# moribots/plen_ml_walk

Measured on NVIDIA B200. Metric: PLEN env-steps/sec, higher is better.
Workload: dtype f32

## Files before the change

### plen_ml_walk_b200/csrc/plen_device.cuh

```cuda
#pragma once

#include <math.h>
#include <stdint.h>

#include "../../include/plen_b200.h"

#ifndef PLEN_HOST_EMU
#define PLEN_DEV __device__ __forceinline__
#define PLEN_DEV_NOINLINE __device__ __noinline__
namespace plen {
PLEN_DEV int lane_id() { return threadIdx.x & 31; }
PLEN_DEV float shfl(float v, int src) { return __shfl_sync(0xffffffffu, v, src); }
PLEN_DEV float shfl4(float v, int src) { return __shfl_sync(0xffffffffu, v, src, 4); }
PLEN_DEV float shfl_up(float v, int d) { return __shfl_up_sync(0xffffffffu, v, d); }
PLEN_DEV float shfl_down(float v, int d) { return __shfl_down_sync(0xffffffffu, v, d); }
PLEN_DEV float shfl_xor(float v, int m) { return __shfl_xor_sync(0xffffffffu, v, m); }
PLEN_DEV unsigned ballot(bool p) { return __ballot_sync(0xffffffffu, p); }
PLEN_DEV unsigned redux_max(unsigned v) { return __reduce_max_sync(0xffffffffu, v); }
PLEN_DEV unsigned redux_or(unsigned v) { return __reduce_or_sync(0xffffffffu, v); }
PLEN_DEV void warp_sync() { __syncwarp(); }
PLEN_DEV float f_as_u_max(float v) { return __uint_as_float(redux_max(__float_as_uint(v))); }
PLEN_DEV void sincos_(float x, float *s, float *c) { sincosf(x, s, c); }
#ifndef PLEN_FAST_RCP
#define PLEN_FAST_RCP 1
#endif
PLEN_DEV float rcp_(float x) {
#if PLEN_FAST_RCP
    float r;
    asm("rcp.approx.ftz.f32 %0, %1;" : "=f"(r) : "f"(x));
    return r;
#else
    return 1.0f / x;
#endif
}
PLEN_DEV unsigned f_bits(float v) { return __float_as_uint(v); }
PLEN_DEV int lowest_bit(unsigned m) { return __ffs((int)m) - 1; }
PLEN_DEV int highest_bit(unsigned m) { return 31 - __clz((int)m); }
PLEN_DEV int popc_(unsigned m) { return __popc(m); }
}
#endif

namespace plen {

enum {
    T_RPJ = 0, T_PPJ = 9, T_AXIS = 12, T_COM = 15, T_MASS = 18, T_INERTIA = 19, T_LOWER = 25, T_UPPER = 26,
    T_CS = 27, T_CE = 28, T_ENVLO = 29, T_ENVHI = 30,
    T_BOX_LANE = 31, T_BOX_C = 32, T_BOX_R = 35, T_BOX_H = 44, T_BOX_REST = 47, T_ROWS = 48
};

enum {
    W_U = 0,
    W_Q = 32,
    W_POS = 32,
    W_MAN = 35,
    W_EPRET = 36,
    W_QUAT = 56,
    W_CNT = 60, W_DS = 61, W_HIST = 62, W_EPT = 63,
    W_LAST = 64,
    W_SUMS = 70,
    W_ITERS = 79,
    W_SPARE = 80
};

struct DevConfig {
    float dt, inv_dt, gravity_z, motor_imp, kp_over_dt, one_minus_kd, linear_damping;
    float mu_lateral, mu_spinning, mu_rolling, restitution, rest_thresh, erp_contact_over_dt, erp_joint_over_dt;
    float linear_slop, warm, hull_margin, vmax, residual_threshold, mu_link;
    float foot_break[2];
    float foot_pts[2][4][3];
    float start_pos[3];
    int foot_lane[2];
    int substeps, reset_ticks, iterations, joint_act, max_episode_steps, auto_reset, link_contacts, n_boxes;
    int sole_manifold, n_hull[2];
    const float *hull;
    float support_tie;
};

enum {
    SR_G = 0,
    SR_B = 960,
    SR_MRHS = 1152, SR_MD = 1184, SR_LDIR = 1216, SR_LRHS = 1248, SR_VSTAR = 1280, SR_Q = 1312,
    SR_CRHS = 1344, SR_CDINV = 1408, SR_CD = 1472,
    SR_PT = 1536,
    SR_LAMC = 1568,
    SR_BASE = 1576,
    SR_WORDS = 1600
};

enum {
    XR_NX = 0,
    XR_ROWS = 16,
    XR_J = 0, XR_B = 32, XR_BB = 64, XR_RHS = 70, XR_DINV = 71, XR_D = 72, XR_ROW_WORDS = 80,
    XR_WORDS = XR_ROWS + 3 * PLEN_MAX_BOX_POINTS * XR_ROW_WORDS
};
#define PLEN_KEY_EXT 125

PLEN_DEV int nth_bit4(unsigned m, int k) {
    int r = -1, c = 0;
#pragma unroll
    for (int b = 0; b < 4; b++) {
        const bool on = (m >> b) & 1u;
        r = (on && c == k) ? b : r;
        c += on ? 1 : 0;
    }
    return r;
}

#ifndef PLEN_HOST_EMU
struct __align__(16) vec4 { float x, y, z, w; };
struct __align__(8) vec2 { float x, y; };
#define PLEN_ALIGN16 __align__(16)
#else
struct vec4 { float x, y, z, w; };
struct vec2 { float x, y; };
#define PLEN_ALIGN16
#endif

#ifndef PLEN_HOST_EMU
PLEN_DEV float gld(const float *p) {
    float v;
    asm("ld.global.f32 %0, [%1];" : "=f"(v) : "l"(p));
    return v;
}
PLEN_DEV vec4 gld4(const float *p) {
    vec4 r;
    asm("ld.global.v4.f32 {%0, %1, %2, %3}, [%4];" : "=f"(r.x), "=f"(r.y), "=f"(r.z), "=f"(r.w) : "l"(p));
    return r;
}
PLEN_DEV int gld_i(const int *p) {
    int v;
    asm("ld.global.s32 %0, [%1];" : "=r"(v) : "l"(p));
    return v;
}
PLEN_DEV int gld_u8(const uint8_t *p) {
    unsigned v;
    asm("ld.global.u8 %0, [%1];" : "=r"(v) : "l"(p));
    return (int)v;
}
#else
PLEN_DEV float gld(const float *p) { return *p; }
PLEN_DEV vec4 gld4(const float *p) { return *reinterpret_cast<const vec4 *>(p); }
PLEN_DEV int gld_i(const int *p) { return *p; }
PLEN_DEV int gld_u8(const uint8_t *p) { return *p; }
#endif

PLEN_DEV void load6(const float *row, float (&o)[6]) {
    const vec4 a = *reinterpret_cast<const vec4 *>(row);
    const vec2 b = *reinterpret_cast<const vec2 *>(row + 4);
    o[0] = a.x; o[1] = a.y; o[2] = a.z; o[3] = a.w; o[4] = b.x; o[5] = b.y;
}

struct PLEN_ALIGN16 WarpScratch {
    float st[96];
    float tw[24][8];
    float kk[24][8];
    float gg[24][8];
    float cb[32];
    float minv[24][32];
    float cp[8][4];
    union {
        float lin[12][12];
        float red[32 * 21];
    };
    float obs[32];
    float xp[PLEN_MAX_BOX_POINTS][8];
    float mn[2][28];
    float mlam[8];
};

struct LaneState {
    float u;
    float q;
    float tgt;
    float lam;
    float pos[3];
    float quat[4];
    unsigned man;
    int iters;
    float fric_s, motor_s, kp_s;
};

PLEN_DEV void mat3_mul(const float *A, const float *B, float *C) {
#pragma unroll
    for (int i = 0; i < 3; i++)
#pragma unroll
        for (int j = 0; j < 3; j++) C[3 * i + j] = A[3 * i] * B[j] + A[3 * i + 1] * B[3 + j] + A[3 * i + 2] * B[6 + j];
}
PLEN_DEV void mat3_vec(const float *A, const float *v, float *o) {
    o[0] = A[0] * v[0] + A[1] * v[1] + A[2] * v[2];
    o[1] = A[3] * v[0] + A[4] * v[1] + A[5] * v[2];
    o[2] = A[6] * v[0] + A[7] * v[1] + A[8] * v[2];
}
PLEN_DEV void cross(const float *a, const float *b, float *o) {
    o[0] = a[1] * b[2] - a[2] * b[1];
    o[1] = a[2] * b[0] - a[0] * b[2];
    o[2] = a[0] * b[1] - a[1] * b[0];
}
PLEN_DEV void quat_to_mat(const float *q, float *R) {
    const float x = q[0], y = q[1], z = q[2], w = q[3];
    R[0] = 1 - 2 * (y * y + z * z); R[1] = 2 * (x * y - w * z); R[2] = 2 * (x * z + w * y);
    R[3] = 2 * (x * y + w * z); R[4] = 1 - 2 * (x * x + z * z); R[5] = 2 * (y * z - w * x);
    R[6] = 2 * (x * z - w * y); R[7] = 2 * (y * z + w * x); R[8] = 1 - 2 * (x * x + y * y);
}
PLEN_DEV float warp_sum(float v) {
#pragma unroll
    for (int m = 16; m > 0; m >>= 1) v += shfl_xor(v, m);
    return v;
}
PLEN_DEV void warp_sum2(float &a, float &b) {
#pragma unroll
    for (int m = 16; m > 0; m >>= 1) { a += shfl_xor(a, m); b += shfl_xor(b, m); }
}

PLEN_DEV void forward_kinematics(const float *tab, int lane, float q, const float *quat, float *Rw, float *pw) {
    float R[9], p[3];
    {
        float s, c;
        sincos_(q, &s, &c);
        const float ax = tab[(T_AXIS + 0) * 32 + lane], ay = tab[(T_AXIS + 1) * 32 + lane], az = tab[(T_AXIS + 2) * 32 + lane];
        const float t = 1.0f - c;
        float Rq[9] = {t * ax * ax + c, t * ax * ay - s * az, t * ax * az + s * ay,
                       t * ax * ay + s * az, t * ay * ay + c, t * ay * az - s * ax,
                       t * ax * az - s * ay, t * ay * az + s * ax, t * az * az + c};
        float Rpj[9];
#pragma unroll
        for (int k = 0; k < 9; k++) Rpj[k] = tab[(T_RPJ + k) * 32 + lane];
        mat3_mul(Rpj, Rq, R);
#pragma unroll
        for (int k = 0; k < 3; k++) p[k] = tab[(T_PPJ + k) * 32 + lane];
    }
    const int cs = (int)tab[T_CS * 32 + lane];
#pragma unroll
    for (int d = 1; d < 8; d <<= 1) {
        float Rp[9], pp[3];
#pragma unroll
        for (int k = 0; k < 9; k++) Rp[k] = shfl_up(R[k], d);
#pragma unroll
        for (int k = 0; k < 3; k++) pp[k] = shfl_up(p[k], d);
        if (lane - d >= cs) {
            float t[3], Rn[9];
            mat3_vec(Rp, p, t);
            p[0] = pp[0] + t[0]; p[1] = pp[1] + t[1]; p[2] = pp[2] + t[2];
            mat3_mul(Rp, R, Rn);
#pragma unroll
            for (int k = 0; k < 9; k++) R[k] = Rn[k];
        }
    }
    float R0[9];
    quat_to_mat(quat, R0);
    mat3_mul(R0, R, Rw);
    mat3_vec(R0, p, pw);
}

PLEN_DEV float clampf(float x, float lo, float hi) { return fminf(fmaxf(x, lo), hi); }

PLEN_DEV void row_entries(int type, const float *a, const float *m, const float *Y, float px, float py, float pz,
                          float &J, float &B) {
    switch (type) {
        case 0: J = a[0] * py - a[1] * px + m[2]; B = Y[0] * py - Y[1] * px + Y[5]; break;
        case 1: J = a[2]; B = Y[2]; break;
        case 2: J = -a[1]; B = -Y[1]; break;
        case 3: J = a[0]; B = Y[0]; break;
        case 4: J = a[0] * pz - a[2] * px - m[1]; B = Y[0] * pz - Y[2] * px - Y[4]; break;
        default: J = a[1] * pz - a[2] * py + m[0]; B = Y[1] * pz - Y[2] * py + Y[3]; break;
    }
}

struct DebugOut { float *minv, *pos, *rot; };

PLEN_DEV_NOINLINE void box_rows(const DevConfig &cfg, const float *tab, WarpScratch &ws, int lane, float vstar, int nx, float *srx);
PLEN_DEV_NOINLINE int box_points(const DevConfig &cfg, const float *tab, WarpScratch &ws, int lane, bool touch, float cz, float rz0,
                                 float rz1, float rz2, int bl, float R0, float R1, float R2, float R3, float R4, float R5, float R6,
                                 float R7, float R8, float p0, float p1, float p2);

PLEN_DEV_NOINLINE void manifold_merge(const DevConfig &cfg, float *mn, float *lam, const float *Rf, const float *pf, const float *pos,
                                      int f, int idx);

PLEN_DEV_NOINLINE unsigned sole_manifold_contacts(const DevConfig &cfg, WarpScratch &ws, int lane, float *man, float pos0, float pos1,
                                                  float pos2, float lam_in, float R0, float R1, float R2, float R3, float R4, float R5,
                                                  float R6, float R7, float R8, float p0, float p1, float p2);

PLEN_DEV void tick_dynamics(const DevConfig &cfg, const float *tab, WarpScratch &ws, LaneState &L, int lane,
                            float *srec, uint8_t *sort_key, const DebugOut *dbg = nullptr, float *srx = nullptr,
                            float *man = nullptr) {
    const bool is_joint = lane >= 6 && lane < 24;
    const int cs = (int)tab[T_CS * 32 + lane], ce = (int)tab[T_CE * 32 + lane];
    float Rw[9], pw[3];
    forward_kinematics(tab, lane, L.q, L.quat, Rw, pw);

    float a[3] = {0, 0, 0}, m[3] = {0, 0, 0};
    if (is_joint) {
        float ax[3] = {tab[(T_AXIS + 0) * 32 + lane], tab[(T_AXIS + 1) * 32 + lane], tab[(T_AXIS + 2) * 32 + lane]};
        mat3_vec(Rw, ax, a);
        cross(pw, a, m);
    } else if (lane < 3) {
        a[lane] = 1.0f;
    } else if (lane < 6) {
        m[lane - 3] = 1.0f;
    }
    if (lane < 24) {
#pragma unroll
        for (int k = 0; k < 3; k++) { ws.tw[lane][k] = a[k]; ws.tw[lane][3 + k] = m[k]; }
    }

    const float mass = tab[T_MASS * 32 + lane];
    float h[3], Ib[6];
    {
        float com[3] = {tab[(T_COM + 0) * 32 + lane], tab[(T_COM + 1) * 32 + lane], tab[(T_COM + 2) * 32 + lane]};
        float c[3];
        mat3_vec(Rw, com, c);
        c[0] += pw[0]; c[1] += pw[1]; c[2] += pw[2];
        const float ixx = tab[(T_INERTIA + 0) * 32 + lane], iyy = tab[(T_INERTIA + 1) * 32 + lane],
                    izz = tab[(T_INERTIA + 2) * 32 + lane], ixy = tab[(T_INERTIA + 3) * 32 + lane],
                    ixz = tab[(T_INERTIA + 4) * 32 + lane], iyz = tab[(T_INERTIA + 5) * 32 + lane];
        float T[9] = {Rw[0] * ixx + Rw[1] * ixy + Rw[2] * ixz, Rw[0] * ixy + Rw[1] * iyy + Rw[2] * iyz, Rw[0] * ixz + Rw[1] * iyz + Rw[2] * izz,
                      Rw[3] * ixx + Rw[4] * ixy + Rw[5] * ixz, Rw[3] * ixy + Rw[4] * iyy + Rw[5] * iyz, Rw[3] * ixz + Rw[4] * iyz + Rw[5] * izz,
                      Rw[6] * ixx + Rw[7] * ixy + Rw[8] * ixz, Rw[6] * ixy + Rw[7] * iyy + Rw[8] * iyz, Rw[6] * ixz + Rw[7] * iyz + Rw[8] * izz};
        const float cc = c[0] * c[0] + c[1] * c[1] + c[2] * c[2];
        Ib[0] = T[0] * Rw[0] + T[1] * Rw[1] + T[2] * Rw[2] + mass * (cc - c[0] * c[0]);
        Ib[1] = T[3] * Rw[3] + T[4] * Rw[4] + T[5] * Rw[5] + mass * (cc - c[1] * c[1]);
        Ib[2] = T[6] * Rw[6] + T[7] * Rw[7] + T[8] * Rw[8] + mass * (cc - c[2] * c[2]);
        Ib[3] = T[0] * Rw[3] + T[1] * Rw[4] + T[2] * Rw[5] - mass * c[0] * c[1];
        Ib[4] = T[0] * Rw[6] + T[1] * Rw[7] + T[2] * Rw[8] - mass * c[0] * c[2];
        Ib[5] = T[3] * Rw[6] + T[4] * Rw[7] + T[5] * Rw[8] - mass * c[1] * c[2];
        h[0] = mass * c[0]; h[1] = mass * c[1]; h[2] = mass * c[2];
    }

    float V0[6];
#pragma unroll
    for (int k = 0; k < 6; k++) V0[k] = shfl(L.u, k);
    float tv[6];
#pragma unroll
    for (int k = 0; k < 3; k++) { tv[k] = is_joint ? a[k] * L.u : 0.0f; tv[3 + k] = is_joint ? m[k] * L.u : 0.0f; }
    float V[6];
#pragma unroll
    for (int k = 0; k < 6; k++) V[k] = tv[k];
#pragma unroll
    for (int d = 1; d < 8; d <<= 1) {
#pragma unroll
        for (int k = 0; k < 6; k++) {
            const float t = shfl_up(V[k], d);
            if (lane - d >= cs) V[k] += t;
        }
    }
#pragma unroll
    for (int k = 0; k < 6; k++) V[k] += V0[k];

    float ab[6];
    {
        float t1[3], t2[3], t3[3];
        cross(V, tv, t1);
        cross(V, tv + 3, t2);
        cross(V + 3, tv, t3);
#pragma unroll
        for (int k = 0; k < 3; k++) { ab[k] = t1[k]; ab[3 + k] = t2[k] + t3[k]; }
#pragma unroll
        for (int d = 1; d < 8; d <<= 1) {
#pragma unroll
            for (int k = 0; k < 6; k++) {
                const float t = shfl_up(ab[k], d);
                if (lane - d >= cs) ab[k] += t;
            }
        }
        float wv[3];
        cross(V0, V0 + 3, wv);
        ab[3] -= wv[0]; ab[4] -= wv[1]; ab[5] -= wv[2] + cfg.gravity_z;
    }

    float F[6];
    {
        float IV[6], Ia[6], t[3], t2[3];
        cross(h, V + 3, t);
        IV[0] = Ib[0] * V[0] + Ib[3] * V[1] + Ib[4] * V[2] + t[0];
        IV[1] = Ib[3] * V[0] + Ib[1] * V[1] + Ib[5] * V[2] + t[1];
        IV[2] = Ib[4] * V[0] + Ib[5] * V[1] + Ib[2] * V[2] + t[2];
        cross(h, V, t);
        IV[3] = mass * V[3] - t[0]; IV[4] = mass * V[4] - t[1]; IV[5] = mass * V[5] - t[2];
        cross(h, ab + 3, t);
        Ia[0] = Ib[0] * ab[0] + Ib[3] * ab[1] + Ib[4] * ab[2] + t[0];
        Ia[1] = Ib[3] * ab[0] + Ib[1] * ab[1] + Ib[5] * ab[2] + t[1];
        Ia[2] = Ib[4] * ab[0] + Ib[5] * ab[1] + Ib[2] * ab[2] + t[2];
        cross(h, ab, t);
        Ia[3] = mass * ab[3] - t[0]; Ia[4] = mass * ab[4] - t[1]; Ia[5] = mass * ab[5] - t[2];
        cross(V, IV, t);
        cross(V + 3, IV + 3, t2);
        F[0] = Ia[0] + t[0] + t2[0]; F[1] = Ia[1] + t[1] + t2[1]; F[2] = Ia[2] + t[2] + t2[2];
        cross(V, IV + 3, t);
        F[3] = Ia[3] + t[0]; F[4] = Ia[4] + t[1]; F[5] = Ia[5] + t[2];
        if (cfg.linear_damping != 0.0f && mass > 0.0f) {
            float c[3] = {h[0] / mass, h[1] / mass, h[2] / mass}, vc[3], fd[3], nd[3];
            cross(V, c, t);
            vc[0] = V[3] + t[0]; vc[1] = V[4] + t[1]; vc[2] = V[5] + t[2];
            const float nv = sqrtf(vc[0] * vc[0] + vc[1] * vc[1] + vc[2] * vc[2]);
            const float k = cfg.linear_damping * mass * (1.0f + nv);
            fd[0] = -k * vc[0]; fd[1] = -k * vc[1]; fd[2] = -k * vc[2];
            cross(c, fd, nd);
            F[0] -= nd[0]; F[1] -= nd[1]; F[2] -= nd[2];
            F[3] -= fd[0]; F[4] -= fd[1]; F[5] -= fd[2];
        }
    }

    float mc = mass, hc[3] = {h[0], h[1], h[2]}, Ic[6] = {Ib[0], Ib[1], Ib[2], Ib[3], Ib[4], Ib[5]};
    float Fc[6] = {F[0], F[1], F[2], F[3], F[4], F[5]};
#pragma unroll
    for (int d = 1; d < 8; d <<= 1) {
        const bool take = is_joint && (lane + d <= ce);
        float t;
        t = shfl_down(mc, d); if (take) mc += t;
#pragma unroll
        for (int k = 0; k < 3; k++) { t = shfl_down(hc[k], d); if (take) hc[k] += t; }
#pragma unroll
        for (int k = 0; k < 6; k++) { t = shfl_down(Ic[k], d); if (take) Ic[k] += t; }
#pragma unroll
        for (int k = 0; k < 6; k++) { t = shfl_down(Fc[k], d); if (take) Fc[k] += t; }
    }
    float mt, ht[3], It[6], Ft[6];
    {
        const bool root = (lane == 0) || (is_joint && lane == cs);
        const unsigned roots = ballot(root);
        const int ord = popc_(roots & ((1u << lane) - 1u)), n_roots = popc_(roots);
        if (root) {
            float *dst = ws.red + 16 * ord;
            dst[0] = mc; dst[1] = hc[0]; dst[2] = hc[1]; dst[3] = hc[2];
#pragma unroll
            for (int k = 0; k < 6; k++) { dst[4 + k] = Ic[k]; dst[10 + k] = Fc[k]; }
        }
        warp_sync();
        float acc[16];
#pragma unroll
        for (int v = 0; v < 16; v++) acc[v] = 0.0f;
        for (int r = 0; r < n_roots; r++) {
#pragma unroll
            for (int q = 0; q < 4; q++) {
                const vec4 x = *reinterpret_cast<const vec4 *>(ws.red + 16 * r + 4 * q);
                acc[4 * q] += x.x; acc[4 * q + 1] += x.y; acc[4 * q + 2] += x.z; acc[4 * q + 3] += x.w;
            }
        }
        mt = acc[0]; ht[0] = acc[1]; ht[1] = acc[2]; ht[2] = acc[3];
#pragma unroll
        for (int k = 0; k < 6; k++) { It[k] = acc[4 + k]; Ft[k] = acc[10 + k]; }
        warp_sync();
    }

    float Cl = 0.0f, fM[6] = {0, 0, 0, 0, 0, 0};
    if (is_joint) {
        Cl = a[0] * Fc[0] + a[1] * Fc[1] + a[2] * Fc[2] + m[0] * Fc[3] + m[1] * Fc[4] + m[2] * Fc[5];
        float t[3];
        cross(hc, m, t);
        fM[0] = Ic[0] * a[0] + Ic[3] * a[1] + Ic[4] * a[2] + t[0];
        fM[1] = Ic[3] * a[0] + Ic[1] * a[1] + Ic[5] * a[2] + t[1];
        fM[2] = Ic[4] * a[0] + Ic[5] * a[1] + Ic[2] * a[2] + t[2];
        cross(hc, a, t);
        fM[3] = mc * m[0] - t[0]; fM[4] = mc * m[1] - t[1]; fM[5] = mc * m[2] - t[2];
    } else if (lane < 6) {
        Cl = Ft[lane];
    }
    ws.cb[lane] = Cl;

    float Mrow[6], Krow[6];
    const int off = lane - cs;
    {
        if (lane < 24) {
#pragma unroll
            for (int k = 0; k < 6; k++) ws.kk[lane][k] = fM[k];
        }
        warp_sync();
#pragma unroll
        for (int d = 0; d < 6; d++) {
            const int j = cs + d;
            float v = (d == off) ? 1.0f : 0.0f;
            if (is_joint && j <= ce) {
                float r6[6];
                if (d <= off) {
                    load6(ws.tw[j], r6);
                    v = r6[0] * fM[0] + r6[1] * fM[1] + r6[2] * fM[2] + r6[3] * fM[3] + r6[4] * fM[4] + r6[5] * fM[5];
                } else {
                    load6(ws.kk[j], r6);
                    v = a[0] * r6[0] + a[1] * r6[1] + a[2] * r6[2] + m[0] * r6[3] + m[1] * r6[4] + m[2] * r6[5];
                }
            }
            Mrow[d] = v;
        }
#pragma unroll
        for (int k = 0; k < 6; k++) Krow[k] = fM[k];
        warp_sync();
    }
#pragma unroll
    for (int k = 0; k < 6; k++) {
        const bool act = is_joint && (cs + k <= ce);
        const int src = act ? cs + k : lane;
        float pr[6], pk[6];
#pragma unroll
        for (int d = 0; d < 6; d++) pr[d] = shfl(Mrow[d], src);
#pragma unroll
        for (int d = 0; d < 6; d++) pk[d] = shfl(Krow[d], src);
        if (act) {
            const float inv = rcp_(pr[k]);
            if (off == k) {
#pragma unroll
                for (int d = 0; d < 6; d++) Mrow[d] = (d == k) ? inv : pr[d] * inv;
#pragma unroll
                for (int d = 0; d < 6; d++) Krow[d] = pk[d] * inv;
            } else {
                const float f = Mrow[k] * inv;
#pragma unroll
                for (int d = 0; d < 6; d++) Mrow[d] = (d == k) ? -f : Mrow[d] - f * pr[d];
#pragma unroll
                for (int d = 0; d < 6; d++) Krow[d] -= f * pk[d];
            }
        }
    }

    {
        int idx = 0;
#pragma unroll
        for (int r = 0; r < 6; r++)
#pragma unroll
            for (int c = r; c < 6; c++) { ws.red[lane * 21 + idx] = is_joint ? fM[r] * Krow[c] : 0.0f; idx++; }
        warp_sync();
        if (lane < 21) {
            float s = 0.0f;
            for (int j = 6; j < 24; j++) s += ws.red[j * 21 + lane];
            ws.red[lane] = s;
        }
    }
    warp_sync();
    float R[6];
    {
        float M00[6][6] = {{It[0], It[3], It[4], 0.0f, -ht[2], ht[1]},
                           {It[3], It[1], It[5], ht[2], 0.0f, -ht[0]},
                           {It[4], It[5], It[2], -ht[1], ht[0], 0.0f},
                           {0.0f, ht[2], -ht[1], mt, 0.0f, 0.0f},
                           {-ht[2], 0.0f, ht[0], 0.0f, mt, 0.0f},
                           {ht[1], -ht[0], 0.0f, 0.0f, 0.0f, mt}};
        float S[6][6];
        int idx = 0;
#pragma unroll
        for (int r = 0; r < 6; r++)
#pragma unroll
            for (int c = r; c < 6; c++) {
                const float v = M00[r][c] - ws.red[idx];
                S[r][c] = v; S[c][r] = v; idx++;
            }
#pragma unroll
        for (int c = 0; c < 6; c++) {
            float v = S[0][c];
#pragma unroll
            for (int r = 1; r < 6; r++) v = (lane == r) ? S[r][c] : v;
            R[c] = v;
        }
#pragma unroll
        for (int k = 0; k < 6; k++) {
            const float inv = rcp_(R[k]);
            float P[6];
#pragma unroll
            for (int j = 0; j < 6; j++) P[j] = shfl((j == k) ? inv : R[j] * inv, k);
            const float f = R[k];
            const bool piv = lane == k;
#pragma unroll
            for (int j = 0; j < 6; j++) {
                const float elim = (j == k) ? -(f * P[k]) : R[j] - f * P[j];
                R[j] = piv ? P[j] : elim;
            }
        }
    }
    warp_sync();
    if (lane < 6) {
#pragma unroll
        for (int k = 0; k < 6; k++) ws.gg[lane][k] = R[k];
    }
    warp_sync();
    float G[6];
    {
        float Si[6][6];
#pragma unroll
        for (int b = 0; b < 6; b++)
#pragma unroll
            for (int c = 0; c < 6; c++) Si[b][c] = ws.gg[b][c];
#pragma unroll
        for (int c = 0; c < 6; c++) {
            float s = 0.0f;
#pragma unroll
            for (int b = 0; b < 6; b++) s += Krow[b] * Si[b][c];
            G[c] = is_joint ? s : 0.0f;
        }
    }
    warp_sync();
    if (lane < 24) {
#pragma unroll
        for (int k = 0; k < 6; k++) { ws.kk[lane][k] = is_joint ? Krow[k] : 0.0f; ws.gg[lane][k] = G[k]; }
    }
    warp_sync();
    if (lane < 24) {
#pragma unroll
        for (int k = 0; k < 6; k++) ws.minv[k][lane] = is_joint ? -G[k] : R[k];
        const float *ggl = &ws.gg[0][is_joint ? 0 : lane];
#pragma unroll 6
        for (int j = 6; j < 24; j++) {
            float r6[6];
            load6(ws.kk[j], r6);
            const float s = G[0] * r6[0] + G[1] * r6[1] + G[2] * r6[2] + G[3] * r6[3] + G[4] * r6[4] + G[5] * r6[5];
            ws.minv[j][lane] = is_joint ? s : -ggl[j * 8];
        }
        if (is_joint) {
#pragma unroll
            for (int d = 0; d < 6; d++)
                if (cs + d <= ce) ws.minv[cs + d][lane] += Mrow[d];
        }
    }
    warp_sync();

    if (dbg != nullptr && lane < 24) {
        if (dbg->minv) for (int j = 0; j < 24; j++) dbg->minv[lane * 24 + j] = ws.minv[j][lane];
        if (dbg->pos) for (int k = 0; k < 3; k++) dbg->pos[lane * 3 + k] = pw[k] + L.pos[k];
        if (dbg->rot) for (int k = 0; k < 9; k++) dbg->rot[lane * 9 + k] = Rw[k];
    }

    float vstar = 0.0f;
    if (lane < 24) {
        float acc = 0.0f;
        for (int j = 0; j < 24; j++) acc += ws.minv[j][lane] * ws.cb[j];
        vstar = clampf(L.u - cfg.dt * acc, -cfg.vmax, cfg.vmax);
    }

    unsigned man_new;
    if (cfg.sole_manifold && man != nullptr) {
        man_new = sole_manifold_contacts(cfg, ws, lane, man, L.pos[0], L.pos[1], L.pos[2], L.lam, Rw[0], Rw[1], Rw[2], Rw[3], Rw[4],
                                         Rw[5], Rw[6], Rw[7], Rw[8], pw[0], pw[1], pw[2]);
        L.man = man_new;
        L.lam = (lane >= 24) ? ws.mlam[lane - 24] : L.lam;
    } else {
        const int i = lane - 24, f = (lane >= 28) ? 1 : 0;
        const int src = cfg.foot_lane[f];
        float Rf[9], pf[3];
#pragma unroll
        for (int k = 0; k < 9; k++) Rf[k] = shfl(Rw[k], src);
#pragma unroll
        for (int k = 0; k < 3; k++) pf[k] = shfl(pw[k], src);
        bool in = false;
        if (lane >= 24) {
            const float *pt = cfg.foot_pts[f][i & 3];
            float w[3];
            mat3_vec(Rf, pt, w);
            w[0] += pf[0]; w[1] += pf[1]; w[2] += pf[2];
            const float dist = (L.pos[2] + w[2]) - cfg.hull_margin;
            in = dist <= cfg.foot_break[f];
            ws.cp[i][0] = w[0]; ws.cp[i][1] = w[1]; ws.cp[i][2] = w[2] - cfg.hull_margin; ws.cp[i][3] = dist;
            const bool was = (L.man >> i) & 1u;
            if (!in || !was) L.lam = 0.0f;
        }
        man_new = ballot(in) >> 24;
        L.man = man_new;
    }
    warp_sync();

    int nx = 0;
    if (cfg.link_contacts && srx != nullptr) {
        const int bl = (int)tab[T_BOX_LANE * 32 + lane];
        const float r20 = shfl(Rw[6], bl), r21 = shfl(Rw[7], bl), r22 = shfl(Rw[8], bl), pz = shfl(pw[2], bl);
        float rz[3], az[3];
#pragma unroll
        for (int k = 0; k < 3; k++) {
            rz[k] = r20 * tab[(T_BOX_R + k) * 32 + lane] + r21 * tab[(T_BOX_R + 3 + k) * 32 + lane] + r22 * tab[(T_BOX_R + 6 + k) * 32 + lane];
            az[k] = rz[k] * tab[(T_BOX_H + k) * 32 + lane];
        }
        const float cz = L.pos[2] + pz + r20 * tab[(T_BOX_C + 0) * 32 + lane] + r21 * tab[(T_BOX_C + 1) * 32 + lane] +
                         r22 * tab[(T_BOX_C + 2) * 32 + lane];
        const bool touch = lane < cfg.n_boxes && cz - (fabsf(az[0]) + fabsf(az[1]) + fabsf(az[2])) <= 0.0f;
        if (ballot(touch))
            nx = box_points(cfg, tab, ws, lane, touch, cz, rz[0], rz[1], rz[2], bl, Rw[0], Rw[1], Rw[2], Rw[3], Rw[4], Rw[5], Rw[6],
                            Rw[7], Rw[8], pw[0], pw[1], pw[2]);
    }
    const bool ext = nx > 0;

    float Y[2][6];
#pragma unroll
    for (int f = 0; f < 2; f++) {
        const int fl = cfg.foot_lane[f], fcs = fl - 5;
#pragma unroll
        for (int k = 0; k < 6; k++) Y[f][k] = 0.0f;
        if ((((man_new >> (4 * f)) & 0xFu) || (f == 0 && ext)) && lane < 24) {
#pragma unroll
            for (int k = 0; k < 6; k++) Y[f][k] = ws.minv[k][lane];
            for (int j = fcs; j <= fl; j++) {
                const float w = ws.minv[j][lane];
                float r6[6];
                load6(ws.tw[j], r6);
#pragma unroll
                for (int k = 0; k < 6; k++) Y[f][k] += w * r6[k];
            }
        }
    }

    float m_dinv = 0.0f, m_rhs = 0.0f, l_rhs = 0.0f, l_dir = 0.0f;
    if (is_joint) {
        const float m_d = ws.minv[lane][lane];
        m_dinv = (m_d > 1.1920929e-7f) ? rcp_(m_d) : 0.0f;
        const float desired = cfg.kp_over_dt * L.kp_s * (L.tgt - L.q) + cfg.one_minus_kd * vstar;
        m_rhs = (m_dinv > 0.0f) ? (desired - vstar) : 0.0f;
        const float lo = tab[T_LOWER * 32 + lane], hi = tab[T_UPPER * 32 + lane];
        const float pen_lo = L.q - lo, pen_hi = hi - L.q;
        if (m_dinv > 0.0f) {
            if (pen_lo <= 0.0f) { l_dir = 1.0f; l_rhs = -pen_lo * cfg.erp_joint_over_dt - vstar; }
            else if (pen_hi <= 0.0f) { l_dir = -1.0f; l_rhs = -pen_hi * cfg.erp_joint_over_dt + vstar; }
        }
    }
    ws.obs[lane] = vstar;
    if (lane < 24) {
#pragma unroll
        for (int k = 0; k < 6; k++) { ws.kk[lane][k] = Y[0][k]; ws.gg[lane][k] = Y[1][k]; }
    }
    warp_sync();
    if (man_new || ext) {
        if (lane < 12) {
            const int f = (lane >= 6) ? 1 : 0, k = lane - 6 * f, fl = cfg.foot_lane[f];
            float acc = 0.0f;
#pragma unroll
            for (int l = 0; l < 6; l++) acc += ws.tw[l][k] * ws.obs[l];
#pragma unroll
            for (int l = 0; l < 6; l++) acc += ws.tw[fl - 5 + l][k] * ws.obs[fl - 5 + l];
            ws.st[W_SPARE + lane] = acc;
        }
        for (int e = lane; e < 144; e += 32) {
            const int row = e / 12, col = e - 12 * row;
            const int fa = row / 6, a6 = row - 6 * fa, fb = col / 6, b6 = col - 6 * fb;
            const float(*Yb)[8] = fb ? ws.gg : ws.kk;
            float acc = Yb[a6][b6];
            const int fl = cfg.foot_lane[fa];
            for (int j = fl - 5; j <= fl; j++) acc += ws.tw[j][a6] * Yb[j][b6];
            ws.lin[row][col] = acc;
        }
        warp_sync();
    }

    {
        const int i = lane;
        const bool ij = i < 18, ic = (i >= 18 && i < 24) || i >= 26;
        const int fa = (i >= 26) ? 1 : 0, a6 = fa ? i - 26 : i - 18;
        const float(*Ya)[8] = fa ? ws.gg : ws.kk;
        float *G = srec + SR_G;
        ws.obs[lane] = m_dinv;
        warp_sync();
        {
            const float *b1 = ij ? &ws.minv[6][6 + i] : (ic ? &Ya[6][a6] : &ws.cb[0]);
            const int st1 = ij ? 32 : (ic ? 8 : 0);
            const bool on1 = ij || ic;
#pragma unroll
            for (int c = 0; c < 18; c++) {
                const float v = b1[c * st1];
                G[c * 32 + lane] = on1 ? v * ws.obs[6 + c] : 0.0f;
            }
        }
        {
            const bool on2 = ij || (ic && (man_new || ext));
            const float *b2 = ij ? &ws.kk[6 + i][0] : (on2 ? &ws.lin[fa * 6 + a6][0] : &ws.cb[0]);
            const int jump = ij ? (int)(&ws.gg[0][0] - &ws.kk[0][0]) - 6 : 0, st2 = on2 ? 1 : 0;
#pragma unroll
            for (int c = 18; c < 30; c++) {
                const int fb = (c >= 24) ? 1 : 0;
                const float v = b2[(c - 18) * st2 + (fb ? jump : 0)];
                G[c * 32 + lane] = on2 ? v : 0.0f;
            }
        }
        const int src = ij ? 6 + i : 0;
        const float s_rhs = shfl(m_rhs, src), s_dinv = shfl(m_dinv, src), s_ldir = shfl(l_dir, src),
                    s_lrhs = shfl(l_rhs, src), s_vs = shfl(vstar, src), s_q = shfl(L.q, src),
                    s_d = shfl(is_joint ? ws.minv[lane][lane] : 0.0f, src);
        float *Bm = srec + SR_B;
        {
            const float *b3 = ij ? &ws.minv[6 + i][0] : (ic ? &Ya[0][a6] : &ws.cb[0]);
            const int st3 = ij ? 1 : (ic ? 8 : 0);
            const float sc3 = ij ? s_dinv : (ic ? 1.0f : 0.0f);
#pragma unroll
            for (int k = 0; k < 6; k++) Bm[k * 32 + lane] = (ij || ic) ? b3[k * st3] * sc3 : 0.0f;
        }
        srec[SR_MRHS + lane] = ij ? s_rhs : 0.0f;
        srec[SR_MD + lane] = (ij && s_dinv > 0.0f) ? s_d : 0.0f;
        srec[SR_LDIR + lane] = ij ? s_ldir : 0.0f;
        srec[SR_LRHS + lane] = ij ? s_lrhs : 0.0f;
        srec[SR_VSTAR + lane] = ij ? s_vs : 0.0f;
        srec[SR_Q + lane] = ij ? s_q : 0.0f;
    }

#pragma unroll
    for (int half = 0; half < 2; half++) {
        const int f = half, g = lane & 7, comp = g - 2;
        const int pb = nth_bit4((man_new >> (4 * f)) & 15u, lane >> 3);
        const int p = 4 * f + (pb < 0 ? 0 : pb);
        const bool valid = comp >= 0 && pb >= 0;
        float rhs = 0.0f, dinv = 0.0f, d = 0.0f;
        if (valid) {
            const float px = ws.cp[p][0], py = ws.cp[p][1], pz = ws.cp[p][2];
            int i0 = comp, i1 = comp, i2 = comp;
            float c0 = 1.0f, c1 = 0.0f, c2 = 0.0f;
            if (comp == 3) { i0 = 1; i1 = 2; i2 = 3; c0 = pz; c1 = -py; c2 = 1.0f; }
            else if (comp == 4) { i0 = 0; i1 = 2; i2 = 4; c0 = -pz; c1 = px; c2 = 1.0f; }
            else if (comp == 5) { i0 = 0; i1 = 1; i2 = 5; c0 = py; c1 = -px; c2 = 1.0f; }
            const int o = 6 * f;
            d = c0 * (c0 * ws.lin[o + i0][o + i0] + c1 * ws.lin[o + i0][o + i1] + c2 * ws.lin[o + i0][o + i2]) +
                c1 * (c0 * ws.lin[o + i1][o + i0] + c1 * ws.lin[o + i1][o + i1] + c2 * ws.lin[o + i1][o + i2]) +
                c2 * (c0 * ws.lin[o + i2][o + i0] + c1 * ws.lin[o + i2][o + i1] + c2 * ws.lin[o + i2][o + i2]);
            dinv = (d > 1.1920929e-7f) ? rcp_(d) : 0.0f;
            const float *vsf = &ws.st[W_SPARE + 6 * f];
            const float v0 = vsf[i0], v1 = vsf[i1], v2 = vsf[i2];
            const float rel = c0 * v0 + c1 * v1 + c2 * v2;
            if (comp == 5) {
                const float pdist = ws.cp[p][3] + cfg.linear_slop;
                float rest = (fabsf(rel) < cfg.rest_thresh) ? 0.0f : cfg.restitution * -rel;
                rest = fmaxf(rest, 0.0f);
                float velerr = rest - rel, poserr = 0.0f;
                if (pdist > 0.0f) velerr -= pdist * cfg.inv_dt; else poserr = -pdist * cfg.erp_contact_over_dt;
                rhs = (poserr + velerr) * dinv;
            } else {
                rhs = -rel * dinv;
                if (comp < 3) {
                    const float mu = (comp == 2) ? cfg.mu_spinning : cfg.mu_rolling;
                    if (!(mu > 0.0f)) { dinv = 0.0f; rhs = 0.0f; d = 0.0f; }
                }
            }
        }
        srec[SR_CRHS + 32 * half + lane] = rhs;
        srec[SR_CDINV + 32 * half + lane] = dinv;
        srec[SR_CD + 32 * half + lane] = d;
    }
    {
        const int q = lane >> 2, pb = nth_bit4((man_new >> (4 * (q >> 2))) & 15u, q & 3);
        srec[SR_PT + lane] = (pb >= 0) ? ws.cp[4 * (q >> 2) + pb][lane & 3] : 0.0f;
        const int q2 = lane & 7, pb2 = nth_bit4((man_new >> (4 * (q2 >> 2))) & 15u, q2 & 3);
        const float lc = shfl(L.lam, 24 + 4 * (q2 >> 2) + (pb2 < 0 ? 0 : pb2));
        if (lane >= 24) srec[SR_LAMC + q2] = (pb2 >= 0) ? lc : 0.0f;
    }
    if (lane < 6) srec[SR_BASE + lane] = vstar;
    if (lane < 3) srec[SR_BASE + 6 + lane] = L.pos[lane];
    if (lane < 4) srec[SR_BASE + 9 + lane] = L.quat[lane];
    if (lane == 0) {
        srec[SR_BASE + 13] = (float)man_new;
        srec[SR_BASE + 14] = L.fric_s;
        srec[SR_BASE + 15] = L.motor_s;
        const int n0 = popc_(man_new & 15u), n1 = popc_((man_new >> 4) & 15u);
        if (sort_key) *sort_key = ext ? (uint8_t)(PLEN_KEY_EXT + nx - 1) : (uint8_t)((n0 > n1 ? n0 : n1) * 25 + n0 * 5 + n1);
    }
    warp_sync();
    if (ext) box_rows(cfg, tab, ws, lane, vstar, nx, srx);
}

PLEN_DEV_NOINLINE unsigned sole_manifold_contacts(const DevConfig &cfg, WarpScratch &ws, int lane, float *man, float pos0, float pos1,
                                                  float pos2, float lam_in, float R0, float R1, float R2, float R3, float R4, float R5,
                                                  float R6, float R7, float R8, float p0, float p1, float p2) {
    const float Rw[9] = {R0, R1, R2, R3, R4, R5, R6, R7, R8}, pw[3] = {p0, p1, p2}, pos[3] = {pos0, pos1, pos2};
    unsigned man_new = 0;
    float lam_out = 0.0f;
    if (lane < 24) { ws.mn[0][lane] = man[lane]; ws.mn[1][lane] = man[24 + lane]; }
    if (lane < 2) ws.mn[lane][24] = man[48 + lane];
    if (lane >= 24) ws.mlam[lane - 24] = lam_in;
    warp_sync();
    int idx2[2];
#pragma unroll
    for (int f = 0; f < 2; f++) {
        const int src = cfg.foot_lane[f];
        const float r6 = shfl(Rw[6], src), r7 = shfl(Rw[7], src), r8 = shfl(Rw[8], src);
        const float *hv = cfg.hull + (size_t)f * PLEN_MAX_HULL * 3;
        const int nh = cfg.n_hull[f];
        float z[PLEN_MAX_HULL / 32];
        float zmin = 3.0e38f;
#pragma unroll
        for (int j = 0; j < PLEN_MAX_HULL / 32; j++) {
            const int i = lane + 32 * j;
            z[j] = 3.0e38f;
            if (i < nh) z[j] = r6 * hv[3 * i] + r7 * hv[3 * i + 1] + r8 * hv[3 * i + 2];
            zmin = fminf(zmin, z[j]);
        }
#pragma unroll
        for (int d = 16; d > 0; d >>= 1) zmin = fminf(zmin, shfl_xor(zmin, d));
        const float zlim = zmin + cfg.support_tie;
        int idx = 0x7fffffff;
#pragma unroll
        for (int j = PLEN_MAX_HULL / 32 - 1; j >= 0; j--)
            if (z[j] <= zlim && lane + 32 * j < nh) idx = lane + 32 * j;
        idx2[f] = 0x7fffffff - (int)redux_max((unsigned)(0x7fffffff - idx));
    }
    {
        const int f = lane & 1, src = cfg.foot_lane[f];
        float Rf[9], pf[3];
#pragma unroll
        for (int k = 0; k < 9; k++) Rf[k] = shfl(Rw[k], src);
#pragma unroll
        for (int k = 0; k < 3; k++) pf[k] = shfl(pw[k], src);
        if (lane < 2) manifold_merge(cfg, ws.mn[f], ws.mlam + 4 * f, Rf, pf, pos, f, f ? idx2[1] : idx2[0]);
        warp_sync();
    }
    {
        const int i = lane - 24, f = (lane >= 28) ? 1 : 0, k = i & 3;
        const int src = cfg.foot_lane[f];
        float Rf[9], pf[3];
#pragma unroll
        for (int q = 0; q < 9; q++) Rf[q] = shfl(Rw[q], src);
#pragma unroll
        for (int q = 0; q < 3; q++) pf[q] = shfl(pw[q], src);
        bool in = false;
        if (lane >= 24) {
            in = k < (int)ws.mn[f][24];
            float w[3] = {0.0f, 0.0f, 0.0f};
            if (in) { mat3_vec(Rf, &ws.mn[f][3 * k], w); w[0] += pf[0]; w[1] += pf[1]; w[2] += pf[2]; }
            ws.cp[i][0] = w[0]; ws.cp[i][1] = w[1]; ws.cp[i][2] = w[2];
            ws.cp[i][3] = in ? (pos[2] + w[2]) - ws.mn[f][12 + 3 * k + 2] : 0.0f;
            lam_out = in ? ws.mlam[i] : 0.0f;
        }
        man_new = ballot(in) >> 24;
    }
    warp_sync();
    if (lane < 24) { man[lane] = ws.mn[0][lane]; man[24 + lane] = ws.mn[1][lane]; }
    if (lane < 2) man[48 + lane] = ws.mn[lane][24];
    warp_sync();
    if (lane >= 24) ws.mlam[lane - 24] = lam_out;
    warp_sync();
    return man_new;
}

PLEN_DEV_NOINLINE void manifold_merge(const DevConfig &cfg, float *mn, float *lam, const float *Rf, const float *pf, const float *pos,
                                      int f, int idx) {
    float *loc = mn, *pln = mn + 12;
    int n = (int)mn[24];
    const float thr = cfg.foot_break[f];
    const float fx = pos[0] + pf[0], fy = pos[1] + pf[1], fz = pos[2] + pf[2];
    if (idx >= 0 && idx < cfg.n_hull[f]) {
        const float *v = cfg.hull + ((size_t)f * PLEN_MAX_HULL + idx) * 3;
        const float la[3] = {v[0] - cfg.hull_margin * Rf[6], v[1] - cfg.hull_margin * Rf[7], v[2] - cfg.hull_margin * Rf[8]};
        float t[3];
        mat3_vec(Rf, la, t);
        const float pa[3] = {fx + t[0], fy + t[1], fz + t[2]};
        const float dist = pa[2];
        if (dist < thr) {
            int slot = -1;
            float nearest = thr * thr;
            for (int k = 0; k < n; k++) {
                const float e0 = loc[3 * k] - la[0], e1 = loc[3 * k + 1] - la[1], e2 = loc[3 * k + 2] - la[2];
                const float dd = e0 * e0 + e1 * e1 + e2 * e2;
                if (dd < nearest) { nearest = dd; slot = k; }
            }
            if (slot < 0) {
                if (n < 4) { slot = n; n = n + 1; lam[slot] = 0.0f; }
                else {
                    int deepest = -1;
                    float maxpen = dist;
                    for (int k = 0; k < 4; k++) {
                        const float zk = fz + Rf[6] * loc[3 * k] + Rf[7] * loc[3 * k + 1] + Rf[8] * loc[3 * k + 2];
                        if (zk < maxpen) { deepest = k; maxpen = zk; }
                    }
                    float best = -1.0f;
                    slot = 0;
                    for (int k = 0; k < 4; k++) {
                        float res = 0.0f;
                        if (k != deepest) {
                            const int o0 = (k == 0) ? 1 : 0, o1 = (k <= 1) ? 2 : 1, o2 = (k <= 2) ? 3 : 2;
                            const float a[3] = {la[0] - loc[3 * o0], la[1] - loc[3 * o0 + 1], la[2] - loc[3 * o0 + 2]};
                            const float b[3] = {loc[3 * o2] - loc[3 * o1], loc[3 * o2 + 1] - loc[3 * o1 + 1], loc[3 * o2 + 2] - loc[3 * o1 + 2]};
                            float c[3];
                            cross(a, b, c);
                            res = c[0] * c[0] + c[1] * c[1] + c[2] * c[2];
                        }
                        if (res > best) { best = res; slot = k; }
                    }
                    lam[slot] = 0.0f;
                }
            }
            loc[3 * slot] = la[0]; loc[3 * slot + 1] = la[1]; loc[3 * slot + 2] = la[2];
            pln[3 * slot] = pa[0]; pln[3 * slot + 1] = pa[1]; pln[3 * slot + 2] = 0.0f;
        }
    }
    for (int k = n - 1; k >= 0; k--) {
        float t[3];
        mat3_vec(Rf, loc + 3 * k, t);
        const float dist = (fz + t[2]) - pln[3 * k + 2];
        const float dx = pln[3 * k] - (fx + t[0]), dy = pln[3 * k + 1] - (fy + t[1]);
        if (dist > thr || dx * dx + dy * dy > thr * thr) {
            const int last = n - 1;
            if (k != last) {
                for (int c = 0; c < 3; c++) { loc[3 * k + c] = loc[3 * last + c]; pln[3 * k + c] = pln[3 * last + c]; }
                lam[k] = lam[last];
            }
            lam[last] = 0.0f;
            n = last;
        }
    }
    mn[24] = (float)n;
}

// ... 166 lines not shown
```

Baseline: 17.75 million.

## Replace warp shuffle broadcasts with vectorized shared-memory staging in dynamics tick

Many warp shuffle broadcasts (joint rows, pivot rows, foot frames, base velocity) are replaced by writing values to per-warp shared scratch and reading them back with vec4/vec2 loads. The spatial-inertia update for the foot contact rows is restructured so that 24 lanes each compute six outputs with vectorized loads instead of a strided 144-element loop. Dynamic lane-indexed register accesses are turned into select chains so they do not spill to local memory. The aim is to cut shuffle count and per-element shared loads. In exchange it adds warp_sync barriers and shared-memory round trips, and it relies on the scratch regions (red, kk) being free at those points.

```diff
diff --git a/plen_ml_walk_b200/csrc/plen_device.cuh b/plen_ml_walk_b200/csrc/plen_device.cuh
--- a/plen_ml_walk_b200/csrc/plen_device.cuh
+++ b/plen_ml_walk_b200/csrc/plen_device.cuh
@@ -149,6 +149,12 @@
     const vec2 b = *reinterpret_cast<const vec2 *>(row + 4);
     o[0] = a.x; o[1] = a.y; o[2] = a.z; o[3] = a.w; o[4] = b.x; o[5] = b.y;
 }
+PLEN_DEV void store6(float *row, float v0, float v1, float v2, float v3, float v4, float v5) {
+    vec4 a; a.x = v0; a.y = v1; a.z = v2; a.w = v3;
+    vec2 b; b.x = v4; b.y = v5;
+    *reinterpret_cast<vec4 *>(row) = a;
+    *reinterpret_cast<vec2 *>(row + 4) = b;
+}
 
 struct PLEN_ALIGN16 WarpScratch {
     float st[96];
@@ -288,19 +294,16 @@
     float Rw[9], pw[3];
     forward_kinematics(tab, lane, L.q, L.quat, Rw, pw);
 
-    float a[3] = {0, 0, 0}, m[3] = {0, 0, 0};
+    float a[3], m[3];
+#pragma unroll
+    for (int k = 0; k < 3; k++) { a[k] = (lane == k) ? 1.0f : 0.0f; m[k] = (lane == 3 + k) ? 1.0f : 0.0f; }
     if (is_joint) {
         float ax[3] = {tab[(T_AXIS + 0) * 32 + lane], tab[(T_AXIS + 1) * 32 + lane], tab[(T_AXIS + 2) * 32 + lane]};
         mat3_vec(Rw, ax, a);
         cross(pw, a, m);
-    } else if (lane < 3) {
-        a[lane] = 1.0f;
-    } else if (lane < 6) {
-        m[lane - 3] = 1.0f;
     }
     if (lane < 24) {
-#pragma unroll
-        for (int k = 0; k < 3; k++) { ws.tw[lane][k] = a[k]; ws.tw[lane][3 + k] = m[k]; }
+        store6(ws.tw[lane], a[0], a[1], a[2], m[0], m[1], m[2]);
     }
 
     const float mass = tab[T_MASS * 32 + lane];
@@ -327,8 +330,7 @@
     }
 
     float V0[6];
-#pragma unroll
-    for (int k = 0; k < 6; k++) V0[k] = shfl(L.u, k);
+    load6(ws.st + W_U, V0);
     float tv[6];
 #pragma unroll
     for (int k = 0; k < 3; k++) { tv[k] = is_joint ? a[k] * L.u : 0.0f; tv[3 + k] = is_joint ? m[k] * L.u : 0.0f; }
@@ -452,8 +454,9 @@
         fM[2] = Ic[4] * a[0] + Ic[5] * a[1] + Ic[2] * a[2] + t[2];
         cross(hc, a, t);
         fM[3] = mc * m[0] - t[0]; fM[4] = mc * m[1] - t[1]; fM[5] = mc * m[2] - t[2];
-    } else if (lane < 6) {
-        Cl = Ft[lane];
+    } else {
+#pragma unroll
+        for (int k = 0; k < 6; k++) Cl = (lane == k) ? Ft[k] : Cl;
     }
     ws.cb[lane] = Cl;
 
@@ -488,12 +491,20 @@
 #pragma unroll
     for (int k = 0; k < 6; k++) {
         const bool act = is_joint && (cs + k <= ce);
-        const int src = act ? cs + k : lane;
+        if (off == k) {
+            float *dst = ws.red + 12 * lane;
+            store6(dst, Mrow[0], Mrow[1], Mrow[2], Mrow[3], Mrow[4], Mrow[5]);
+            store6(dst + 6, Krow[0], Krow[1], Krow[2], Krow[3], Krow[4], Krow[5]);
+        }
+        warp_sync();
         float pr[6], pk[6];
-#pragma unroll
-        for (int d = 0; d < 6; d++) pr[d] = shfl(Mrow[d], src);
-#pragma unroll
-        for (int d = 0; d < 6; d++) pk[d] = shfl(Krow[d], src);
+        {
+            const float *srcp = ws.red + 12 * (act ? cs + k : 6 + k);
+            const vec4 x0 = *reinterpret_cast<const vec4 *>(srcp), x1 = *reinterpret_cast<const vec4 *>(srcp + 4),
+                       x2 = *reinterpret_cast<const vec4 *>(srcp + 8);
+            pr[0] = x0.x; pr[1] = x0.y; pr[2] = x0.z; pr[3] = x0.w; pr[4] = x1.x; pr[5] = x1.y;
+            pk[0] = x1.z; pk[1] = x1.w; pk[2] = x2.x; pk[3] = x2.y; pk[4] = x2.z; pk[5] = x2.w;
+        }
         if (act) {
             const float inv = rcp_(pr[k]);
             if (off == k) {
@@ -511,6 +522,7 @@
         }
     }
 
+    warp_sync();
     {
         int idx = 0;
 #pragma unroll
@@ -553,8 +565,13 @@
         for (int k = 0; k < 6; k++) {
             const float inv = rcp_(R[k]);
             float P[6];
-#pragma unroll
-            for (int j = 0; j < 6; j++) P[j] = shfl((j == k) ? inv : R[j] * inv, k);
+            if (lane == k) {
+#pragma unroll
+                for (int j = 0; j < 6; j++) P[j] = (j == k) ? inv : R[j] * inv;
+                store6(ws.kk[k], P[0], P[1], P[2], P[3], P[4], P[5]);
+            }
+            warp_sync();
+            load6(ws.kk[k], P);
             const float f = R[k];
             const bool piv = lane == k;
 #pragma unroll
@@ -565,10 +582,7 @@
         }
     }
     warp_sync();
-    if (lane < 6) {
-#pragma unroll
-        for (int k = 0; k < 6; k++) ws.gg[lane][k] = R[k];
-    }
+    if (lane < 6) store6(ws.gg[lane], R[0], R[1], R[2], R[3], R[4], R[5]);
     warp_sync();
     float G[6];
     {
@@ -586,21 +600,19 @@
         }
     }
     warp_sync();
+    if (lane < 24) store6(ws.kk[lane], is_joint ? Krow[0] : 0.0f, is_joint ? Krow[1] : 0.0f, is_joint ? Krow[2] : 0.0f,
+                          is_joint ? Krow[3] : 0.0f, is_joint ? Krow[4] : 0.0f, is_joint ? Krow[5] : 0.0f);
+    warp_sync();
     if (lane < 24) {
 #pragma unroll
-        for (int k = 0; k < 6; k++) { ws.kk[lane][k] = is_joint ? Krow[k] : 0.0f; ws.gg[lane][k] = G[k]; }
-    }
-    warp_sync();
-    if (lane < 24) {
-#pragma unroll
         for (int k = 0; k < 6; k++) ws.minv[k][lane] = is_joint ? -G[k] : R[k];
-        const float *ggl = &ws.gg[0][is_joint ? 0 : lane];
+        if (is_joint) store6(ws.minv[lane], -G[0], -G[1], -G[2], -G[3], -G[4], -G[5]);
 #pragma unroll 6
         for (int j = 6; j < 24; j++) {
             float r6[6];
             load6(ws.kk[j], r6);
             const float s = G[0] * r6[0] + G[1] * r6[1] + G[2] * r6[2] + G[3] * r6[3] + G[4] * r6[4] + G[5] * r6[5];
-            ws.minv[j][lane] = is_joint ? s : -ggl[j * 8];
+            if (is_joint) ws.minv[j][lane] = s;
         }
         if (is_joint) {
 #pragma unroll
@@ -631,21 +643,29 @@
         L.lam = (lane >= 24) ? ws.mlam[lane - 24] : L.lam;
     } else {
         const int i = lane - 24, f = (lane >= 28) ? 1 : 0;
-        const int src = cfg.foot_lane[f];
-        float Rf[9], pf[3];
-#pragma unroll
-        for (int k = 0; k < 9; k++) Rf[k] = shfl(Rw[k], src);
-#pragma unroll
-        for (int k = 0; k < 3; k++) pf[k] = shfl(pw[k], src);
+        const int fw = (lane == cfg.foot_lane[0]) ? 0 : ((lane == cfg.foot_lane[1]) ? 1 : -1);
+        if (fw >= 0) {
+            vec4 *dst = reinterpret_cast<vec4 *>(&ws.kk[0][0] + 16 * fw);
+            vec4 x;
+            x.x = Rw[0]; x.y = Rw[1]; x.z = Rw[2]; x.w = Rw[3]; dst[0] = x;
+            x.x = Rw[4]; x.y = Rw[5]; x.z = Rw[6]; x.w = Rw[7]; dst[1] = x;
+            x.x = Rw[8]; x.y = pw[0]; x.z = pw[1]; x.w = pw[2]; dst[2] = x;
+        }
+        warp_sync();
         bool in = false;
         if (lane >= 24) {
+            const vec4 *fr = reinterpret_cast<const vec4 *>(&ws.kk[0][0] + 16 * f);
+            const vec4 x0 = fr[0], x1 = fr[1], x2 = fr[2];
+            const float Rf[9] = {x0.x, x0.y, x0.z, x0.w, x1.x, x1.y, x1.z, x1.w, x2.x}, pf[3] = {x2.y, x2.z, x2.w};
             const float *pt = cfg.foot_pts[f][i & 3];
             float w[3];
             mat3_vec(Rf, pt, w);
             w[0] += pf[0]; w[1] += pf[1]; w[2] += pf[2];
             const float dist = (L.pos[2] + w[2]) - cfg.hull_margin;
             in = dist <= cfg.foot_break[f];
-            ws.cp[i][0] = w[0]; ws.cp[i][1] = w[1]; ws.cp[i][2] = w[2] - cfg.hull_margin; ws.cp[i][3] = dist;
+            vec4 c4;
+            c4.x = w[0]; c4.y = w[1]; c4.z = w[2] - cfg.hull_margin; c4.w = dist;
+            *reinterpret_cast<vec4 *>(ws.cp[i]) = c4;
             const bool was = (L.man >> i) & 1u;
             if (!in || !was) L.lam = 0.0f;
         }
@@ -673,7 +693,9 @@
     }
     const bool ext = nx > 0;
 
-    float Y[2][6];
+    float Y[2][6], mb[6];
+#pragma unroll
+    for (int k = 0; k < 6; k++) mb[k] = (man_new || ext) && lane < 24 ? ws.minv[k][lane] : 0.0f;
 #pragma unroll
     for (int f = 0; f < 2; f++) {
         const int fl = cfg.foot_lane[f], fcs = fl - 5;
@@ -681,7 +703,7 @@
         for (int k = 0; k < 6; k++) Y[f][k] = 0.0f;
         if ((((man_new >> (4 * f)) & 0xFu) || (f == 0 && ext)) && lane < 24) {
 #pragma unroll
-            for (int k = 0; k < 6; k++) Y[f][k] = ws.minv[k][lane];
+            for (int k = 0; k < 6; k++) Y[f][k] = mb[k];
             for (int j = fcs; j <= fl; j++) {
                 const float w = ws.minv[j][lane];
                 float r6[6];
@@ -707,28 +729,39 @@
     }
     ws.obs[lane] = vstar;
     if (lane < 24) {
-#pragma unroll
-        for (int k = 0; k < 6; k++) { ws.kk[lane][k] = Y[0][k]; ws.gg[lane][k] = Y[1][k]; }
+        store6(ws.kk[lane], Y[0][0], Y[0][1], Y[0][2], Y[0][3], Y[0][4], Y[0][5]);
+        store6(ws.gg[lane], Y[1][0], Y[1][1], Y[1][2], Y[1][3], Y[1][4], Y[1][5]);
     }
     warp_sync();
     if (man_new || ext) {
         if (lane < 12) {
             const int f = (lane >= 6) ? 1 : 0, k = lane - 6 * f, fl = cfg.foot_lane[f];
+            float vb[6];
+            load6(ws.obs, vb);
             float acc = 0.0f;
 #pragma unroll
-            for (int l = 0; l < 6; l++) acc += ws.tw[l][k] * ws.obs[l];
+            for (int l = 0; l < 6; l++) acc += ws.tw[l][k] * vb[l];
 #pragma unroll
             for (int l = 0; l < 6; l++) acc += ws.tw[fl - 5 + l][k] * ws.obs[fl - 5 + l];
             ws.st[W_SPARE + lane] = acc;
         }
-        for (int e = lane; e < 144; e += 32) {
-            const int row = e / 12, col = e - 12 * row;
-            const int fa = row / 6, a6 = row - 6 * fa, fb = col / 6, b6 = col - 6 * fb;
+        if (lane < 24) {
+            const int fa = (lane >= 12) ? 1 : 0, col = lane - 12 * fa, fb = (col >= 6) ? 1 : 0, b6 = col - 6 * fb;
             const float(*Yb)[8] = fb ? ws.gg : ws.kk;
-            float acc = Yb[a6][b6];
-            const int fl = cfg.foot_lane[fa];
-            for (int j = fl - 5; j <= fl; j++) acc += ws.tw[j][a6] * Yb[j][b6];
-            ws.lin[row][col] = acc;
+            const int j0 = cfg.foot_lane[fa] - 5;
+            float acc[6];
+#pragma unroll
+            for (int a = 0; a < 6; a++) acc[a] = Yb[a][b6];
+#pragma unroll
+            for (int t = 0; t < 6; t++) {
+                float s6[6];
+                load6(ws.tw[j0 + t], s6);
+                const float y = Yb[j0 + t][b6];
+#pragma unroll
+                for (int a = 0; a < 6; a++) acc[a] += s6[a] * y;
+            }
+#pragma unroll
+            for (int a = 0; a < 6; a++) ws.lin[6 * fa + a][col] = acc[a];
         }
         warp_sync();
     }
@@ -745,22 +778,40 @@
             const float *b1 = ij ? &ws.minv[6][6 + i] : (ic ? &Ya[6][a6] : &ws.cb[0]);
             const int st1 = ij ? 32 : (ic ? 8 : 0);
             const bool on1 = ij || ic;
+            float sc[18];
+            {
+                const vec2 s2 = *reinterpret_cast<const vec2 *>(ws.obs + 6);
+                sc[0] = s2.x; sc[1] = s2.y;
+#pragma unroll
+                for (int q = 0; q < 4; q++) {
+                    const vec4 s4 = *reinterpret_cast<const vec4 *>(ws.obs + 8 + 4 * q);
+                    sc[2 + 4 * q] = s4.x; sc[3 + 4 * q] = s4.y; sc[4 + 4 * q] = s4.z; sc[5 + 4 * q] = s4.w;
+                }
+            }
 #pragma unroll
             for (int c = 0; c < 18; c++) {
                 const float v = b1[c * st1];
-                G[c * 32 + lane] = on1 ? v * ws.obs[6 + c] : 0.0f;
+                G[c * 32 + lane] = on1 ? v * sc[c] : 0.0f;
             }
         }
         {
             const bool on2 = ij || (ic && (man_new || ext));
             const float *b2 = ij ? &ws.kk[6 + i][0] : (on2 ? &ws.lin[fa * 6 + a6][0] : &ws.cb[0]);
-            const int jump = ij ? (int)(&ws.gg[0][0] - &ws.kk[0][0]) - 6 : 0, st2 = on2 ? 1 : 0;
-#pragma unroll
-            for (int c = 18; c < 30; c++) {
-                const int fb = (c >= 24) ? 1 : 0;
-                const float v = b2[(c - 18) * st2 + (fb ? jump : 0)];
-                G[c * 32 + lane] = on2 ? v : 0.0f;
-            }
+            const float *b2b = ij ? &ws.gg[6 + i][0] : b2 + 6;
+            float v2[12];
+            {
+                float r6[6];
+                load6(b2, r6);
+#pragma unroll
+                for (int k = 0; k < 6; k++) v2[k] = r6[k];
+#pragma unroll
+                for (int k = 0; k < 3; k++) {
+                    const vec2 x = *reinterpret_cast<const vec2 *>(b2b + 2 * k);
+                    v2[6 + 2 * k] = x.x; v2[7 + 2 * k] = x.y;
+                }
+            }
+#pragma unroll
+            for (int c = 18; c < 30; c++) G[c * 32 + lane] = on2 ? v2[c - 18] : 0.0f;
         }
         const int src = ij ? 6 + i : 0;
         const float s_rhs = shfl(m_rhs, src), s_dinv = shfl(m_dinv, src), s_ldir = shfl(l_dir, src),
@@ -831,8 +882,8 @@
         if (lane >= 24) srec[SR_LAMC + q2] = (pb2 >= 0) ? lc : 0.0f;
     }
     if (lane < 6) srec[SR_BASE + lane] = vstar;
-    if (lane < 3) srec[SR_BASE + 6 + lane] = L.pos[lane];
-    if (lane < 4) srec[SR_BASE + 9 + lane] = L.quat[lane];
+    if (lane < 3) srec[SR_BASE + 6 + lane] = ws.st[W_POS + lane];
+    if (lane < 4) srec[SR_BASE + 9 + lane] = ws.st[W_QUAT + lane];
     if (lane == 0) {
         srec[SR_BASE + 13] = (float)man_new;
         srec[SR_BASE + 14] = L.fric_s;
```

New measurement: 18.33 million, median of 6. +3.3%, better.
